# Ray0089/geometric-aware-dense-matching

Measured on AMD Instinct MI355X. Metric: rgbd_crops_per_sec_geomatch_fwd, higher is better.
Workload: dtype bf16x3/f32acc

## Files before the change

### geometric_aware_dense_matching_amd/csrc/gdm_image.hip

```cpp
#include "gdm_common.h"
#include "gdm_packed_act.h"

namespace {

__global__ __launch_bounds__(256) void upsample_bilinear_kernel(const float* __restrict__ in, int H, int W, int OH, int OW,
                                                                float rh, float rw, float* __restrict__ out)
{
    const long plane = blockIdx.y;
    const int qpr = (OW + 3) >> 2;
    const int q = blockIdx.x * 256 + threadIdx.x;
    if (q >= qpr * OH) return;
    const int oy = q / qpr;
    const int ox0 = (q - oy * qpr) * 4;
    const float sy = rh * (float)oy;
    const int y0 = (int)sy;
    const int y1 = y0 + (y0 < H - 1 ? 1 : 0);
    const float ly = sy - (float)y0, hy = 1.f - ly;
    const float* r0 = in + (plane * H + y0) * (long)W;
    const float* r1 = in + (plane * H + y1) * (long)W;
    float v[4];
#pragma unroll
    for (int j = 0; j < 4; ++j) {
        const int ox = min(ox0 + j, OW - 1);
        const float sx = rw * (float)ox;
        const int x0 = (int)sx;
        const int x1 = x0 + (x0 < W - 1 ? 1 : 0);
        const float lx = sx - (float)x0, hx = 1.f - lx;
        v[j] = hy * (hx * r0[x0] + lx * r0[x1]) + ly * (hx * r1[x0] + lx * r1[x1]);
    }
    float* o = out + (plane * OH + oy) * (long)OW + ox0;
    if (ox0 + 3 < OW && (((uintptr_t)o) & 15) == 0) {
        *reinterpret_cast<float4*>(o) = make_float4(v[0], v[1], v[2], v[3]);
    } else {
        for (int j = 0; j < 4 && ox0 + j < OW; ++j) o[j] = v[j];
    }
}

__device__ __forceinline__ void src_range(int i, int n_in, int n_out, float r, int& lo, int& hi)
{
    if (r <= 0.f) { lo = 0; hi = n_out - 1; return; }
    lo = max(0, (int)floorf((float)(i - 1) / r) - 1);
    hi = min(n_out - 1, (int)ceilf((float)(i + 1) / r) + 1);
}

__device__ __forceinline__ float tap_weight(int o, int i, int n_in, float r)
{
    const float sp = r * (float)o;
    const int i0 = min((int)sp, n_in - 1);
    const int i1 = i0 + (i0 < n_in - 1 ? 1 : 0);
    const float l = sp - (float)i0;
    return (i0 == i ? 1.f - l : 0.f) + (i1 == i ? l : 0.f);
}
// ... 528 lines not shown
            const int c = i - r * pw;
            const float* src = zb + (long)min(ys0 + r, H - 1) * W + min(xs0 + c, W - 1);
#pragma unroll
            for (int ch = 0; ch < 4; ++ch)
#pragma unroll
                for (int tap = 0; tap < 9; ++tap) patch[ch][tap][r][c] = src[((long)tap * Cout + ch) * plane_sz];
        }
        __syncthreads();
        if (live) {
#pragma unroll
            for (int dy = -1; dy <= 1; ++dy) {
                const int yy = oy + dy;
                if (yy < 0 || yy >= OH) continue;
                const float sy = rh * (float)yy;
                const int y0 = min((int)sy, H - 1);
                const float ly = sy - (float)y0, hy = 1.f - ly;
#pragma unroll
                for (int dx = -1; dx <= 1; ++dx) {
                    const int xx = ox + dx;
                    if (xx < 0 || xx >= OW) continue;
                    const int tap = (dy + 1) * 3 + (dx + 1);
                    const float sx = rw * (float)xx;
                    const int x0 = min((int)sx, W - 1);
                    const float lx = sx - (float)x0, hx = 1.f - lx;
                    const int xo = x0 - xs0, yo = y0 - ys0;
#pragma unroll
                    for (int ch = 0; ch < 4; ++ch) {
                        const float* r0 = &patch[ch][tap][yo][0];
                        const float* r1 = r0 + (U8_PW + 2);
                        const float top = fmaf(lx, r0[xo + 1], hx * r0[xo]);
                        const float bot = fmaf(lx, r1[xo + 1], hx * r1[xo]);
                        acc[4 * pass + ch] = fmaf(ly, bot, fmaf(hy, top, acc[4 * pass + ch]));
                    }
                }
            }
        }
    }
    if (!live) return;
    float v[8];
#pragma unroll
    for (int ch = 0; ch < 8; ++ch) {
        float o = acc[ch] * scale[c0 + ch] + shift[c0 + ch];
        if (ACT == 1) o = fmaxf(o, 0.f);
        if (ACT == 2) o = o > 0.f ? o : o * slope;
        v[ch] = o;
        out[(((long)b * Cout + c0 + ch) * OH + oy) * OW + ox] = o;
    }
    if (ypk) {
        const gdm_packed_map pm{Cout, OH, OW};
        gdm_packed_store8(ypk + pm.granule(b, c0 / GDM_PK_CHUNK, (c0 % GDM_PK_CHUNK) / 8, oy, ox), 0, pm.lo(), v);
    }
}

struct PspMaps {
    const float* y[4];
    int s[4];
    float sy[4], sx[4];
};

__global__ __launch_bounds__(256) void psp_combine_kernel(const float* __restrict__ g, PspMaps maps, const float* __restrict__ bias,
                                                          int C, int H, int W, float* __restrict__ out)
{
    const long plane = blockIdx.y;
    const int c = (int)(plane % C);
    const int hw = H * W;
    const float bc = bias ? bias[c] : 0.f;
    __shared__ float pm[4][64];
    {
        const int k = threadIdx.x >> 6, j = threadIdx.x & 63;
        if (j < maps.s[k] * maps.s[k]) pm[k][j] = maps.y[k][plane * maps.s[k] * maps.s[k] + j];
        __syncthreads();
    }
    for (int i0 = (blockIdx.x * 256 + threadIdx.x) * 4; i0 < hw; i0 += gridDim.x * 1024) {
        int oy = i0 / W, ox = i0 - oy * W;
        float v[4];
        const bool vec = i0 + 3 < hw;
        if (vec) {
            const float4 gv = *reinterpret_cast<const float4*>(g + plane * hw + i0);
            v[0] = gv.x; v[1] = gv.y; v[2] = gv.z; v[3] = gv.w;
        }
#pragma unroll
        for (int e = 0; e < 4; ++e) {
            if (i0 + e < hw) {
                float acc = (vec ? v[e] : g[plane * hw + i0 + e]) + bc;
#pragma unroll
                for (int k = 0; k < 4; ++k) {
                    const int S = maps.s[k];
                    const float* m = &pm[k][0];
                    const float fy = maps.sy[k] * (float)oy, fx = maps.sx[k] * (float)ox;
                    const int y0 = min((int)fy, S - 1), x0 = min((int)fx, S - 1);
                    const int y1 = y0 + (y0 < S - 1 ? 1 : 0), x1 = x0 + (x0 < S - 1 ? 1 : 0);
                    const float ly = fy - (float)y0, lx = fx - (float)x0;
                    acc += (1.f - ly) * ((1.f - lx) * m[y0 * S + x0] + lx * m[y0 * S + x1]) + ly * ((1.f - lx) * m[y1 * S + x0] + lx * m[y1 * S + x1]);
                }
                v[e] = fmaxf(acc, 0.f);
            }
            if (++ox == W) { ox = 0; ++oy; }
        }
        if (vec) *reinterpret_cast<float4*>(out + plane * hw + i0) = make_float4(v[0], v[1], v[2], v[3]);
        else
            for (int e = 0; e < 4 && i0 + e < hw; ++e) out[plane * hw + i0 + e] = v[e];
    }
}

__global__ __launch_bounds__(256) void psp_combine8_kernel(const float* __restrict__ g, PspMaps maps, const float* __restrict__ bias,
                                                           int C, int H, int W, float* __restrict__ out, unsigned char* __restrict__ ypk)
// ... 310 lines not shown
    GDM_CHECK_ARG(((uintptr_t)x & 15) == 0, "gdm_affine_act_maxk_hip: x must be 16-byte aligned");
    dim3 grid(gdm_cdiv(n, 256), (unsigned)planes);
    hipStream_t s = (hipStream_t)stream;
    gdm_dispatch_int<3>(act, [&](auto A) {
        hipLaunchKernelGGL(affine_act_maxk_kernel<decltype(A)::value>, grid, dim3(256), 0, s, x, scale, shift, C, n, K / 4, slope, out);
    });
    return gdm_launch_status("affine_act_maxk_kernel");
}

extern "C" int gdm_prelu1_hip(const float* x, const float* slope, long n, float* y, void* stream)
{
    GDM_CHECK_ARG(x && slope && y, "gdm_prelu1_hip: NULL pointer");
    GDM_CHECK_ARG(n >= 4 && n % 4 == 0 && (((uintptr_t)x | (uintptr_t)y) & 15) == 0, "gdm_prelu1_hip: n=%ld must be a multiple of 4 and the pointers 16-byte aligned", n);
    long blocks = gdm_cdiv(n / 4, 256);
    if (blocks > 8192) blocks = 8192;
    hipLaunchKernelGGL(prelu1_fwd_kernel, dim3((unsigned)blocks), dim3(256), 0, (hipStream_t)stream, (const float4*)x, slope, n / 4, (float4*)y);
    return gdm_launch_status("prelu1_fwd_kernel");
}

extern "C" int gdm_prelu1_bwd_hip(const float* x, const float* grad_out, const float* slope, long n, float* grad_x, float* grad_slope, void* stream)
{
    GDM_CHECK_ARG(x && grad_out && slope && grad_x && grad_slope, "gdm_prelu1_bwd_hip: NULL pointer");
    GDM_CHECK_ARG(n >= 4 && n % 4 == 0 && (((uintptr_t)x | (uintptr_t)grad_out | (uintptr_t)grad_x) & 15) == 0, "gdm_prelu1_bwd_hip: n=%ld must be a multiple of 4 and the pointers 16-byte aligned", n);
    long blocks = gdm_cdiv(n / 4, 256);
    if (blocks > 4096) blocks = 4096;
    hipLaunchKernelGGL(prelu1_bwd_kernel, dim3((unsigned)blocks), dim3(256), 0, (hipStream_t)stream, (const float4*)x, (const float4*)grad_out, slope,
                       n / 4, (float4*)grad_x, grad_slope);
    return gdm_launch_status("prelu1_bwd_kernel");
}

extern "C" int gdm_affine_act_hip(const float* x, const float* scale, const float* shift, const float* res, const float* res_scale,
                                  const float* res_shift, long planes, int C, long inner, int act, float slope, float* y, void* stream)
{
    GDM_CHECK_ARG(x && scale && shift && y, "gdm_affine_act_hip: NULL pointer");
    GDM_CHECK_ARG(planes >= 1 && planes <= 65535 && C >= 1 && inner >= 4 && inner % 4 == 0, "gdm_affine_act_hip: planes=%ld C=%d inner=%ld (inner %% 4 == 0, planes <= 65535)", planes, C, inner);
    GDM_CHECK_ARG(act >= 0 && act <= 2, "gdm_affine_act_hip: act=%d", act);
    GDM_CHECK_ARG((((uintptr_t)x | (uintptr_t)y | (uintptr_t)res) & 15) == 0, "gdm_affine_act_hip: pointers must be 16-byte aligned");
    const long inner4 = inner / 4;
    int gx = gdm_cdiv(inner4, 256);
    if (gx > 64) gx = 64;
    dim3 grid(gx, (unsigned)planes);
    hipStream_t s = (hipStream_t)stream;
    const bool has = res != nullptr, aff = res_scale != nullptr && res_shift != nullptr;
    gdm_dispatch_int<3>(act, [&](auto A) {
        gdm_dispatch_int<3>(!has ? 0 : aff ? 2 : 1, [&](auto R) {
            constexpr int RM = decltype(R)::value;
            hipLaunchKernelGGL((affine_act_kernel<decltype(A)::value, RM != 0, RM == 2>), grid, dim3(256), 0, s, x, scale, shift, res, res_scale,
                               res_shift, C, inner4, slope, y);
        });
    });
    return gdm_launch_status("affine_act_kernel");
}

extern "C" int gdm_upconv3x3_gather2_hip(const float* z, const float* scale, const float* shift, int B, int Cout, int H, int W,
                                         int OH, int OW, int act, float slope, float* out, void* outpk, void* stream)
{
    GDM_CHECK_ARG(z && scale && shift && out && outpk, "gdm_upconv3x3_gather2_hip: NULL pointer");
    GDM_CHECK_ARG(B >= 1 && Cout >= 8 && (long)B * (Cout / 8) <= 65535 && H >= 1 && W >= 1 && OH >= 1 && OW >= 1,
                  "gdm_upconv3x3_gather2_hip: bad shape B=%d Cout=%d %dx%d -> %dx%d", B, Cout, H, W, OH, OW);
    GDM_CHECK_ARG(act >= 0 && act <= 2 && gdm_packed_out_ok(Cout, outpk),
                  "gdm_upconv3x3_gather2_hip: act=%d / packed output needs Cout = 64 or a multiple of 128 and a 16-byte aligned buffer (Cout=%d)", act, Cout);
    const float rh = scale_ac(H, OH), rw = scale_ac(W, OW);
    GDM_CHECK_ARG((int)(rh * (U8_H + 1)) + 3 <= U8_PH && (int)(rw * (U8_W + 1)) + 3 <= U8_PW,
                  "gdm_upconv3x3_gather2_hip: scale factors %g x %g too large for the LDS tile (the x2 stages of PSPUpsample fit)", rh, rw);
    hipStream_t s = (hipStream_t)stream;
    dim3 grid(gdm_cdiv(OW, U8_W), gdm_cdiv(OH, U8_H), B * (Cout / 8));
    gdm_dispatch_int<3>(act, [&](auto A) {
        hipLaunchKernelGGL(upconv3x3_gather8_kernel<decltype(A)::value>, grid, dim3(256), 0, s, z, scale, shift, Cout, H, W, OH, OW, rh, rw, slope, out,
                           (unsigned char*)outpk);
    });
    return gdm_launch_status("upconv3x3_gather8_kernel");
}

extern "C" int gdm_upconv3x3_gather_hip(const float* z, const float* scale, const float* shift, int B, int Cout, int H, int W,
                                        int OH, int OW, int act, float slope, float* out, void* stream)
{
    GDM_CHECK_ARG(z && scale && shift && out, "gdm_upconv3x3_gather_hip: NULL pointer");
    GDM_CHECK_ARG(B >= 1 && Cout >= 1 && (long)B * Cout <= 65535 && H >= 1 && W >= 1 && OH >= 1 && OW >= 1,
                  "gdm_upconv3x3_gather_hip: bad shape B=%d Cout=%d %dx%d -> %dx%d", B, Cout, H, W, OH, OW);
    GDM_CHECK_ARG(act >= 0 && act <= 2, "gdm_upconv3x3_gather_hip: act=%d", act);
    hipStream_t s = (hipStream_t)stream;
    const float rh = scale_ac(H, OH), rw = scale_ac(W, OW);
    const bool lds_ok = (int)(rh * (UT_H + 1)) + 3 <= UP_PH && (int)(rw * (UT_W + 1)) + 3 <= UP_PW && (long)B * Cout <= 65535;
    if (lds_ok) {
        dim3 grid(gdm_cdiv(OW, UT_W), gdm_cdiv(OH, UT_H), B * Cout);
        gdm_dispatch_int<3>(act, [&](auto A) {
            hipLaunchKernelGGL(upconv3x3_gather_lds_kernel<decltype(A)::value>, grid, dim3(256), 0, s, z, scale, shift, Cout, H, W, OH, OW, rh, rw, slope, out);
        });
        return gdm_launch_status("upconv3x3_gather_lds_kernel");
    }
    const int quads = ((OW + 3) / 4) * OH;
    dim3 grid(gdm_cdiv(quads, 256), B * Cout);
    gdm_dispatch_int<3>(act, [&](auto A) {
        hipLaunchKernelGGL(upconv3x3_gather_kernel<decltype(A)::value>, grid, dim3(256), 0, s, z, scale, shift, Cout, H, W, OH, OW, rh, rw, slope, out);
    });
    return gdm_launch_status("upconv3x3_gather_kernel");
}

extern "C" int gdm_upconv3x3_gather_bwd_hip(const float* grad_out, int B, int Cout, int H, int W, int OH, int OW, float* grad_z, void* stream)
{
    GDM_CHECK_ARG(grad_out && grad_z, "gdm_upconv3x3_gather_bwd_hip: NULL pointer");
    GDM_CHECK_ARG(B >= 1 && Cout >= 1 && H >= 1 && W >= 1 && OH >= 1 && OW >= 1 && (long)B * 9 * Cout <= 65535,
                  "gdm_upconv3x3_gather_bwd_hip: bad shape B=%d Cout=%d (B*9*Cout <= 65535)", B, Cout);
    const float rh = scale_ac(H, OH), rw = scale_ac(W, OW);
    if (rh > 0.f && rw > 0.f && (int)ceilf((TL + 1) / rh) + 7 <= UB_P && (int)ceilf((TL + 1) / rw) + 7 <= UB_P) {
        dim3 grid3(gdm_cdiv(H, TL) * gdm_cdiv(W, TL), (unsigned)(B * Cout));
        hipLaunchKernelGGL(upconv3x3_gather_bwd_lds_kernel, grid3, dim3(256), 0, (hipStream_t)stream, grad_out, Cout, H, W, OH, OW, rh, rw, grad_z);
        return gdm_launch_status("upconv3x3_gather_bwd_lds_kernel");
    }
    dim3 grid(gdm_cdiv(H, TL) * gdm_cdiv(W, TL), (unsigned)(B * 9 * Cout));
    hipLaunchKernelGGL(upconv3x3_gather_bwd_kernel, grid, dim3(256), 0, (hipStream_t)stream, grad_out, Cout, H, W, OH, OW,
                       scale_ac(H, OH), scale_ac(W, OW), grad_z);
    return gdm_launch_status("upconv3x3_gather_bwd_kernel");
}

extern "C" int gdm_psp_combine2_hip(const float* g, const float* y1, int s1, const float* y2, int s2, const float* y3, int s3,
                                    const float* y4, int s4, const float* bias, int B, int C, int H, int W, float* out, void* outpk,
                                    void* stream)
{
    GDM_CHECK_ARG(g && y1 && y2 && y3 && y4 && out, "gdm_psp_combine2_hip: NULL pointer");
    GDM_CHECK_ARG(B >= 1 && C >= 1 && (long)B * C <= 65535 && H >= 1 && W >= 1 && s1 >= 1 && s2 >= 1 && s3 >= 1 && s4 >= 1,
                  "gdm_psp_combine2_hip: bad shape");
    GDM_CHECK_ARG(s1 <= 8 && s2 <= 8 && s3 <= 8 && s4 <= 8, "gdm_psp_combine2_hip: prior maps up to 8x8 (the reference uses 1, 2, 3, 6)");
    PspMaps maps;
    maps.y[0] = y1; maps.y[1] = y2; maps.y[2] = y3; maps.y[3] = y4;
    maps.s[0] = s1; maps.s[1] = s2; maps.s[2] = s3; maps.s[3] = s4;
    for (int k = 0; k < 4; ++k) {
        maps.sy[k] = H > 1 ? (float)(maps.s[k] - 1) / (float)(H - 1) : 0.f;
        maps.sx[k] = W > 1 ? (float)(maps.s[k] - 1) / (float)(W - 1) : 0.f;
    }
    GDM_CHECK_ARG(((long)H * W) % 4 == 0 && (((uintptr_t)g | (uintptr_t)out) & 15) == 0, "gdm_psp_combine2_hip: H*W must be a multiple of 4 and the maps 16-byte aligned");
    int gx = gdm_cdiv((long)H * W, 1024);
    if (gx > 16) gx = 16;
    if (outpk) {
        GDM_CHECK_ARG(W % 4 == 0 && gdm_packed_out_ok(C, outpk),
                      "gdm_psp_combine2_hip: packed output needs C = 64 or a multiple of 128, W %% 4 == 0 and a 16-byte aligned buffer (C=%d W=%d)", C, W);
        hipLaunchKernelGGL(psp_combine8_kernel, dim3(gx, B * C / 8), dim3(256), 0, (hipStream_t)stream, g, maps, bias, C, H, W, out,
// ... 116 lines not shown
```

### geometric_aware_dense_matching_amd/ops.py

```python
import collections
import ctypes
import functools
import os

import torch

from . import _lib, settings
from ._lib import KnnJob, call, check
from .derived import derived

MATCH_BF16X3 = _lib.GDM_MATCH_BF16X3
MATCH_F32 = _lib.GDM_MATCH_F32


def _stream():
    return torch.cuda.current_stream().cuda_stream


_side_streams = {}


def side_stream(device, which=0):
    key = (device.index if device.index is not None else torch.cuda.current_device(), which)
    st = _side_streams.get(key)
# ... 946 lines not shown
        return None
    group = bn.process_group if bn.process_group is not None else dist.group.WORLD
    return group if dist.get_world_size(group) >= settings.SYNCBN_MIN_WORLD else None


def bn_train_supported(x, bn):
    if not (settings.USE_FUSED_BN_TRAIN and bn.training and x.is_cuda and x.dtype == torch.float32 and x.dim() >= 3 and x.is_contiguous()):
        return False
    if type(bn) not in (torch.nn.BatchNorm1d, torch.nn.BatchNorm2d) and not (settings.USE_FUSED_SYNCBN and type(bn) is torch.nn.SyncBatchNorm):
        return False
    if not bn.affine or bn.momentum is None or not bn.track_running_stats:
        return False
    B, C = x.shape[0], x.shape[1]
    inner = x.numel() // max(B * C, 1)
    return B * C <= 65535 and inner >= 4 and inner % 4 == 0 and x.data_ptr() % 16 == 0 and B * inner > 1


def batch_norm_act_train(x, bn, act=ACT_NONE, slope=0.0):
    y = _BatchNormAct.apply(x, bn.weight, bn.bias, bn.running_mean, bn.running_var, bn.eps, bn.momentum, act, slope, _sync_group(bn))
    if bn.num_batches_tracked is not None:
        if _bn_counters is not None:
            _bn_counters.append(bn.num_batches_tracked)
        else:
            bn.num_batches_tracked.add_(1)
    return y


_bn_counters = None


class batched_bn_counters:

    def __enter__(self):
        global _bn_counters
        self.prev, _bn_counters = _bn_counters, []
        return self

    def __exit__(self, *exc):
        global _bn_counters
        pending, _bn_counters = _bn_counters, self.prev
        if pending:
            torch._foreach_add_(pending, 1)
        return False


def upconv3x3_gather(z, scale, shift, cout, out_size, act=ACT_NONE, slope=0.0, packed=False):
    z = _dev(z, torch.float32, "z")
    B, c9, H, W = z.shape
    assert c9 == 9 * cout
    OH, OW = int(out_size[0]), int(out_size[1])
    out = torch.empty((B, cout, OH, OW), dtype=torch.float32, device=z.device)
    if packed and packed_out_supported(B, cout, OH, OW, grid_groups=True) and (OH, OW) == (2 * H, 2 * W):
        opk = _packed_out(B, cout, OH, OW, z.device)
        call("gdm_upconv3x3_gather2_hip", z, scale, shift, B, cout, H, W, OH, OW, act, float(slope), out, opk.buf)
        return carry_packed(out, opk)
    call("gdm_upconv3x3_gather_hip", z, scale, shift, B, cout, H, W, OH, OW, act, float(slope), out)
    return out


def upconv_fused64_pack_weight(weight):
    w = _dev(weight.detach(), torch.float32, "weight")
    if tuple(w.shape) != (64, 64, 3, 3):
        raise ValueError("upconv_fused64_pack_weight: weight must be [64,64,3,3], got %s" % (tuple(w.shape),))
    L = _lib.lib()
    wpk = torch.empty(L.gdm_upconv_fused64_weight_bytes(), dtype=torch.uint8, device=w.device)
    call("gdm_upconv_fused64_pack_weight_hip", w, wpk)
    return wpk


def upconv_fused64(x, wpk, scale, shift, out_size, act=0, slope=0.0):
    x = _dev(x, torch.float32, "x")
    B, C, H, W = x.shape
    OH, OW = int(out_size[0]), int(out_size[1])
    out = torch.empty((B, C, OH, OW), dtype=torch.float32, device=x.device)
    call("gdm_upconv_fused64_hip", x, wpk, scale, shift, B, C, H, W, OH, OW, act, float(slope), out)
    return out


class _UpconvGather(torch.autograd.Function):

    @staticmethod
    def forward(ctx, z, bias, cout, OH, OW):
        z = z.contiguous()
        B, c9, H, W = z.shape
        ones = torch.ones(cout, dtype=torch.float32, device=z.device)
        shift = bias.detach().contiguous() if bias is not None else torch.zeros(cout, dtype=torch.float32, device=z.device)
        out = torch.empty((B, cout, OH, OW), dtype=torch.float32, device=z.device)
        call("gdm_upconv3x3_gather_hip", z, ones, shift, B, cout, H, W, OH, OW, ACT_NONE, 0.0, out)
        ctx.shape = (B, cout, H, W, OH, OW)
        ctx.has_bias = bias is not None
        return out

    @staticmethod
    def backward(ctx, go):
        B, cout, H, W, OH, OW = ctx.shape
        go = go.contiguous()
        gz = torch.empty((B, 9 * cout, H, W), dtype=torch.float32, device=go.device)
        call("gdm_upconv3x3_gather_bwd_hip", go, B, cout, H, W, OH, OW, gz)
        return gz, (channel_sum(go) if ctx.has_bias else None), None, None, None


def upconv3x3_gather_train(z, bias, cout, out_size):
    z = _dev(z, torch.float32, "z")
    assert z.shape[1] == 9 * cout
    return _UpconvGather.apply(z, bias, cout, int(out_size[0]), int(out_size[1]))


def wx(w2d, x3):
    if torch.is_grad_enabled() and (w2d.requires_grad or x3.requires_grad) and x3.is_cuda and x3.dtype == torch.float32:
        return _WxTrain.apply(x3.contiguous(), w2d.contiguous())
    return torch.bmm(w2d.unsqueeze(0).expand(x3.shape[0], -1, -1), x3)


OPERAND_LIMIT = 1 << 31


def operands_fit(*nbytes):
    return all(0 < n < OPERAND_LIMIT for n in nbytes)


def _require_fit(who, what, args, act_bytes, weight_bytes=None):
    if not operands_fit(act_bytes, *(() if weight_bytes is None else (weight_bytes,))):
        raise ValueError("%s: %s needs packed activations of %d bytes%s; a packed operand must be above 0 and below 2 GiB (%d bytes)"
                         % (who, what % args, act_bytes, "" if weight_bytes is None else " and packed weights of %d bytes" % weight_bytes,
                            OPERAND_LIMIT))


def _map_bytes(B, C, H, W):
    return _lib.lib().gdm_conv3x3_act_bytes(B, C, H, W)


def _wgrad_parts(nchunk, tiles):
    parts = 1
    for d in range(1, nchunk + 1):
        if nchunk % d == 0 and d * tiles <= 320 and nchunk // d >= 4:
            parts = d
    return parts


def _wgrad_packed(who, x, go, taps, parts=None):
    B, Cin, Cout = x.shape[0], x.shape[1], go.shape[1]
# ... 1260 lines not shown
```

### geometric_aware_dense_matching_amd/settings.py

```python
import os


def _flag(name, default="1"):
    return os.environ.get(name, default) != "0"


USE_MFMA_CONV = _flag("GDM_MFMA_CONV")
USE_MFMA_CONV_TRAIN = _flag("GDM_MFMA_CONV_TRAIN")
USE_MFMA_GEMM = _flag("GDM_MFMA_GEMM")
USE_FUSED_UPCONV = _flag("GDM_FUSED_UPCONV")
USE_LOWRES_UPCONV_TRAIN = _flag("GDM_LOWRES_UPCONV_TRAIN")
USE_SPLIT_PSP_TRAIN = _flag("GDM_SPLIT_PSP_TRAIN")
USE_FUSED_LFA = _flag("GDM_FUSED_LFA")
USE_GROUPED_SPLINE = _flag("GDM_GROUPED_SPLINE")
USE_FUSED_BN_TRAIN = _flag("GDM_FUSED_BN_TRAIN")
USE_FUSED_SYNCBN = _flag("GDM_FUSED_SYNCBN")
USE_FUSED_MATCH_LOSS = _flag("GDM_FUSED_MATCH_LOSS")
USE_SIDE_STREAMS = _flag("GDM_SIDE_STREAMS", "0")
USE_SPARSE_FINAL = _flag("GDM_SPARSE_FINAL")
USE_FUSED_HEADS = _flag("GDM_FUSED_HEADS")
USE_MFMA_STRIDED = _flag("GDM_MFMA_STRIDED")
USE_POINTWISE = _flag("GDM_POINTWISE")
USE_OWN_STEM = _flag("GDM_OWN_STEM")
USE_GEMM_CONV1X1_TRAIN = _flag("GDM_GEMM_CONV1X1_TRAIN")
USE_MFMA_WGRAD = _flag("GDM_MFMA_WGRAD")
USE_MFMA_GEMM_TRAIN = _flag("GDM_MFMA_GEMM_TRAIN")
USE_GATHERED_FINAL = _flag("GDM_GATHERED_FINAL")
USE_DIRECT_WGRAD = _flag("GDM_DIRECT_WGRAD")
USE_FUSED_ADAM = _flag("GDM_FUSED_ADAM")
USE_POINTWISE_TRAIN = _flag("GDM_POINTWISE_TRAIN")
USE_POINT_CHAIN = _flag("GDM_POINT_CHAIN")
USE_PSP_JOBS = _flag("GDM_PSP_JOBS")
USE_PACKED_PRODUCERS = _flag("GDM_PACKED_PRODUCERS")
MESH_FORK_LATE = os.environ.get("GDM_MESH_FORK_LATE", "1") != "0"
PACK_MESH_ROWS = os.environ.get("GDM_PACK_MESH_ROWS", "1") != "0"
SPLINE_LDS_WEIGHTS = os.environ.get("GDM_SPLINE_LDS_WEIGHTS", "1") != "0"
HEADS_MATCH_ROWS = os.environ.get("GDM_HEADS_MATCH_ROWS", "1") != "0"
SIDE_PARTS = os.environ.get("GDM_SIDE_PARTS", "mesh,point,pyr").split(",")
STATIC_MATCH_ROWS = _flag("GDM_STATIC_MATCH_ROWS", "0")
UPCONV_MIN_CIN = int(os.environ.get("GDM_UPCONV_MIN_CIN", "0"))
SYNCBN_MIN_WORLD = 2

ALL_SWITCHES = ("USE_MFMA_CONV", "USE_MFMA_CONV_TRAIN", "USE_MFMA_GEMM", "USE_FUSED_UPCONV", "USE_LOWRES_UPCONV_TRAIN",
                "USE_SPLIT_PSP_TRAIN", "USE_FUSED_LFA", "USE_GROUPED_SPLINE", "USE_FUSED_BN_TRAIN", "USE_FUSED_SYNCBN",
                "USE_FUSED_MATCH_LOSS", "USE_SIDE_STREAMS", "USE_SPARSE_FINAL", "USE_FUSED_HEADS", "USE_MFMA_STRIDED", "USE_POINTWISE", "USE_OWN_STEM", "USE_GEMM_CONV1X1_TRAIN", "USE_MFMA_WGRAD", "USE_MFMA_GEMM_TRAIN", "USE_GATHERED_FINAL", "USE_DIRECT_WGRAD", "USE_PSP_JOBS", "USE_POINT_CHAIN", "USE_POINTWISE_TRAIN")
SPLIT_BF16_SWITCHES = ("USE_MFMA_CONV", "USE_MFMA_GEMM", "USE_FUSED_UPCONV", "USE_SPARSE_FINAL", "USE_FUSED_HEADS", "USE_MFMA_STRIDED",
                       "USE_OWN_STEM")
```

### include/gdm.h

```cpp
#ifndef GDM_H
#define GDM_H

#include <stddef.h>
#include <stdint.h>

#ifdef __cplusplus
extern "C" {
#endif

#define GDM_EINVAL (-1)
#define GDM_ENOMEM (-2)

const char* gdm_last_error(void);
int gdm_version(void);


void gdm_knn_batch(const float* batch_data, size_t batch_size, size_t npts, size_t dim,
                   const float* queries, size_t nqueries, size_t K, long* batch_indices);

int gdm_knn_batch_hip(const float* support, const float* query, int B, int S, int Q, int K,
                      int32_t* idx, float* d2, void* stream);

typedef struct gdm_knn_job {
    const float* support;
// ... 151 lines not shown
                         const int32_t* best_idx, const uint8_t* mask, int B, int N, int M, double* out, void* stream);

int gdm_kabsch_solve_hip(const double* stats, int B, int min_points, float* RT, uint8_t* valid, void* stream);

int gdm_kabsch_stats_w_hip(const float* scene_xyz, long scene_bstride, int pt_stride, int ch_stride, const float* model_xyz,
                           const int32_t* best_idx, const float* target, const float* weight, const uint8_t* mask, int B, int N,
                           int M, double* out, int32_t* count, void* stream);
int gdm_kabsch_solve_w_hip(const double* stats, const int32_t* count, int B, int min_points, float* RT, uint8_t* valid, void* stream);

#define GDM_RANSAC_MAX_H 4096
size_t gdm_ransac_workspace_bytes(int B, int N, int H);
int gdm_ransac_pose_hip(const float* scene_xyz, long scene_bstride, int pt_stride, int ch_stride, const float* model_xyz,
                        const int32_t* best_idx, const uint8_t* mask, const double* stats, int B, int N, int M, int H,
                        float match_err, double fix_percent, uint32_t seed, int min_points, void* workspace, size_t workspace_bytes,
                        float* RT, uint8_t* valid, int32_t* counts, int32_t* winner, void* stream);

size_t gdm_consensus_workspace_bytes(int B, int N, int seeds);
int gdm_consensus_pose_hip(const float* scene_xyz, long scene_bstride, int pt_stride, int ch_stride, const float* model_xyz,
                           const int32_t* best_idx, const uint8_t* mask, int B, int N, int M, int seeds, float tau, float inlier_dist,
                           int min_points, void* workspace, size_t workspace_bytes, float* RT, uint8_t* valid, int32_t* score,
                           int32_t* degree, int32_t* seed_idx, float* hyp_RT, int32_t* counts, int32_t* winner, void* stream);

int gdm_icp_transform_hip(const float* scene_xyz, long scene_bstride, int pt_stride, int ch_stride, const float* RT, int B, int N,
                          float* query, void* stream);
int gdm_icp_update_hip(const float* scene_xyz, long scene_bstride, int pt_stride, int ch_stride, const float* model_xyz,
                       const int32_t* nn, const float* d2, const uint8_t* mask, int B, int N, int M, float reject_dist,
                       double tolerance, int min_points, float* RT, uint8_t* active, int32_t* iters, double* err, void* stream);

int gdm_icp_plane_update_hip(const float* scene_nrm, long scene_bstride, int pt_stride, int ch_stride, const float* query,
                             const float* model_xyz, const float* model_nrm, const int32_t* nn, const float* d2, const uint8_t* mask,
                             int B, int N, int M, float reject_dist, double normal_gate, double huber_delta, double tolerance,
                             int min_points, double pivot_min, float* RT, uint8_t* active, int32_t* iters, double* err,
                             int32_t* status, int32_t* n_pairs, void* stream);

#define GDM_TARGETS_MIN_M 4
size_t gdm_targets_workspace_bytes(int B, int N, int M);
int gdm_hpr_visible_hip(const float* model_xyz, long model_bstride, const float* RT, const float* cam_center, int B, int M,
                        void* workspace, size_t workspace_bytes, double* flipped, uint8_t* visible, void* stream);
int gdm_pose_targets_hip(const float* cld, long cld_bstride, int pt_stride, int ch_stride, const uint8_t* labels, const float* RT,
                         const float* model_xyz, long model_bstride, const uint8_t* visible, int B, int N, int M, double dist_thresh,
                         void* workspace, size_t workspace_bytes, uint8_t* labels_out, int32_t* match_idx, uint8_t* visible_flag,
                         uint8_t* valid, void* stream);

int gdm_affine_act_maxk_hip(const float* x, const float* scale, const float* shift, long planes, int C, long n, int K, int act,
                            float slope, float* out, void* stream);

int gdm_prelu1_hip(const float* x, const float* slope, long n, float* y, void* stream);
int gdm_prelu1_bwd_hip(const float* x, const float* grad_out, const float* slope, long n, float* grad_x, float* grad_slope, void* stream);

int gdm_affine_act_hip(const float* x, const float* scale, const float* shift, const float* res, const float* res_scale,
                       const float* res_shift, long planes, int C, long inner, int act, float slope, float* y, void* stream);

int gdm_upconv3x3_gather_hip(const float* z, const float* scale, const float* shift, int B, int Cout, int H, int W,
                             int OH, int OW, int act, float slope, float* out, void* stream);
int gdm_upconv3x3_gather2_hip(const float* z, const float* scale, const float* shift, int B, int Cout, int H, int W,
                              int OH, int OW, int act, float slope, float* out, void* outpk, void* stream);
int gdm_upconv3x3_gather_bwd_hip(const float* grad_out, int B, int Cout, int H, int W, int OH, int OW, float* grad_z, void* stream);
size_t gdm_upconv_fused64_weight_bytes(void);
int gdm_upconv_fused64_pack_weight_hip(const float* w, void* wpk, void* stream);
int gdm_upconv_fused64_hip(const float* x, const void* wpk, const float* scale, const float* shift, int B, int C, int H, int W,
                           int OH, int OW, int act, float slope, float* out, void* stream);

int gdm_psp_combine2_hip(const float* g, const float* y1, int s1, const float* y2, int s2, const float* y3, int s3,
                         const float* y4, int s4, const float* bias, int B, int C, int H, int W, float* out, void* outpk, void* stream);
int gdm_gather_add_affine_act2_hip(const float* x, const float* t, const int32_t* idx, const float* scale, const float* shift,
                                   int B, int C, int n, int m, int act, float slope, float* y, void* y_packed, int W, void* stream);
int gdm_conv1x1_gather_add_act2_hip(const float* x, const float* wt, const float* t, const int32_t* idx, const float* scale,
                                    const float* shift, int B, int C, int n, long m, int act, float slope, int pixel_major,
                                    float* y, void* stream);
int gdm_conv64_gather_add_act_mfma2_hip(const float* x, const void* wpk, const float* t, const int32_t* idx, const float* scale,
                                        const float* shift, int B, int n, long m, int act, float slope, int pixel_major,
                                        int t_point_major, float* y, void* ypk, int W, void* stream);
int gdm_conv64_gather_add_final_hip(const float* x, const void* wpk, const float* t, const int32_t* idx, const float* scale,
                                    const float* shift, int B, int n, long m, int act, float slope, const float* wft,
                                    const float* fbias, float* out, void* stream);

size_t gdm_conv3x3_act_bytes(int B, int Cin, int H, int W);
size_t gdm_conv3x3_weight_bytes(int Cout, int Cin);
int gdm_conv3x3_pack_weight_hip(const float* w, int Cout, int Cin, void* wpk, void* stream);
int gdm_conv3x3_pack_act_hip(const float* x, int B, int Cin, int H, int W, void* xpk, void* stream);
int gdm_conv3x3_packed_hip(const void* xpk, const void* wpk, const float* scale, const float* shift, const float* res,
                           int B, int Cin, int Cout, int H, int W, int act, float* out, void* stream);
int gdm_conv3x3_strided_hip(const void* xpk, const void* wpk, const float* scale, const float* shift, const float* res,
                            int B, int Cin, int Cout, int H, int W, int stride, int act, float* out, void* outpk, void* stream);
int gdm_conv1x1_strided_hip(const void* xpk, const void* wpk, const float* scale, const float* shift,
                            int B, int Cin, int Cout, int H, int W, int stride, int act, float* out, void* stream);
int gdm_conv1x1_gather_add_hip(const void* xpk, const void* wpk, const int32_t* gidx, const float* gt, int gn, const float* scale,
                               const float* shift, int B, int Cin, int Cout, int H, int W, int act, float* out, void* outpk, void* stream);

int gdm_affine_relu_maxpool_hip(const float* x, const float* scale, const float* shift, int B, int C, int H, int W, float* y, void* stream);
int gdm_conv1x1_logsoftmax_hip(const float* x, const float* w, const float* bias, int B, int C, long hw, float* out, void* stream);
int gdm_pack_rows64_hip(const float* w, int R, void* out, void* stream);
int gdm_upconv_final_points_hip(const float* xpm, const int32_t* choose, const void* wpk, const float* scale, const float* shift,
                                int act, float slope, const void* wfpk, const float* fbias, int B, int H, int W, int OH, int OW,
                                int N, float* out, void* stream);
int gdm_psp_pools_hip(const float* x, long planes, int H, int W, float* o1, float* o2, float* o3, float* o6, void* stream);
int gdm_psp_pools_bwd_hip(const float* g1, const float* g2, const float* g3, const float* g6, long planes, int H, int W,
                          float* grad_x, void* stream);

size_t gdm_conv1x1_weight_bytes(int Cout, int Cin);
int gdm_conv1x1_pack_weight_hip(const float* w, int Cout, int Cin, void* wpk, void* stream);
int gdm_conv_pack_weight_dgrad_hip(const float* w, int Cout, int Cin, int taps, void* wpk, void* stream);
int gdm_conv1x1_packed_hip(const void* xpk, const void* wpk, const float* scale, const float* shift,
                           int B, int Cin, int Cout, int H, int W, int act, int pixel_major, float* out, void* stream);

int gdm_depth_to_xyz_hip(const float* depth, const float* K, const int32_t* origin, int B, int H, int W, int S,
                         float* out, void* stream);

#define GDM_NORMALS_MAX_K 64
// ... 155 lines not shown
```

Baseline: 5407.

## Add full-row LDS tiled upconv3x3 gather kernels for exact x2 upsampling

Adds two new upconv3x3 gather kernels that stage whole input row windows for all nine taps into LDS using vectorized 16-byte loads. The next channel group's loads are software-pipelined behind the current compute, and a dispatcher picks these kernels for exact 2x upsampling with small widths. The packed eight-channel path is enabled by a default-on setting. The non-packed path always passes 0, so the four-channel rows kernel never runs from Python. This aims to cut redundant global gathers and per-tile halo overhead, at the cost of large LDS use per block, which may limit occupancy.

```diff
diff --git a/geometric_aware_dense_matching_amd/csrc/gdm_image.hip b/geometric_aware_dense_matching_amd/csrc/gdm_image.hip
--- a/geometric_aware_dense_matching_amd/csrc/gdm_image.hip
+++ b/geometric_aware_dense_matching_amd/csrc/gdm_image.hip
@@ -1,3 +1,4 @@
+#include <climits>
 #include "gdm_common.h"
 #include "gdm_packed_act.h"
 
@@ -632,6 +633,237 @@
     }
 }
 
+#ifdef __HIP_DEVICE_COMPILE__
+#define UR_NO_PACKED_F32 __attribute__((target("no-packed-fp32-ops")))
+#else
+#define UR_NO_PACKED_F32
+#endif
+__device__ __forceinline__ UR_NO_PACKED_F32 void ur_barrier()
+{
+    __builtin_amdgcn_fence(__ATOMIC_RELEASE, "workgroup");
+    __builtin_amdgcn_s_barrier();
+    __builtin_amdgcn_fence(__ATOMIC_ACQUIRE, "workgroup");
+}
+constexpr int UR_LAST = 1 << 30;
+
+template <int NLD, int NT, int NCH>
+__device__ __forceinline__ UR_NO_PACKED_F32 void rowfill_plan(int ph, int H, int W, int ys0, int Cout, unsigned plane_sz, int stride, unsigned (&g)[NLD], int (&l)[NLD])
+{
+    const int W4 = W >> 2, n = 9 * NCH * ph * W4;
+    const unsigned inv_w4 = ((1u << 20) + W4 - 1) / W4, inv_ph = ((1u << 20) + ph - 1) / ph;
+#pragma unroll
+    for (int k = 0; k < NLD; ++k) {
+        const int i = threadIdx.x + k * NT;
+        const int row = (int)(((unsigned)i * inv_w4) >> 20), c4 = i - row * W4;
+        const int p = (int)(((unsigned)row * inv_ph) >> 20), r = row - p * ph;
+        const int tap = p / NCH, ch = p - tap * NCH;
+        const bool is = i < n;
+        g[k] = is ? (unsigned)(tap * Cout + ch) * plane_sz + (unsigned)(min(ys0 + r, H - 1) * W + 4 * c4) : 0u;
+        l[k] = is ? (row * stride + 4 * c4) | (c4 == W4 - 1 ? UR_LAST : 0) : -1;
+    }
+}
+template <int NLD>
+__device__ __forceinline__ UR_NO_PACKED_F32 void rowfill_load(const float* __restrict__ zq, const unsigned (&g)[NLD], gdm_f32x4 (&v)[NLD])
+{
+#pragma unroll
+    for (int k = 0; k < NLD; ++k) v[k] = *reinterpret_cast<const gdm_f32x4*>(zq + g[k]);
+}
+template <int NLD>
+__device__ __forceinline__ UR_NO_PACKED_F32 void rowfill_store(float* patch, const int (&l)[NLD], const gdm_f32x4 (&v)[NLD])
+{
+#pragma unroll
+    for (int k = 0; k < NLD; ++k) {
+        if (l[k] >= 0) {
+            const int o = l[k] & (UR_LAST - 1);
+            *reinterpret_cast<gdm_f32x4*>(patch + o) = v[k];
+            if (l[k] & UR_LAST) patch[o + 4] = v[k][3];
+        }
+    }
+}
+__device__ __forceinline__ UR_NO_PACKED_F32 void rowfill_window(int oy_t, int TH, int H, int OH, float rh, int& ys0, int& ph)
+{
+    ys0 = min((int)(rh * (float)max(oy_t - 1, 0)), H - 1);
+    ph = min((int)(rh * (float)min(oy_t + TH, OH - 1)), H - 1) - ys0 + 2;
+}
+
+constexpr int R8_TH = 8, R8_PH = 7, R8_NLD = 8, R8_MAXW = 32, R8_LDS = 36 * R8_PH * (R8_MAXW + 4);
+
+template <int ACT>
+__global__ __launch_bounds__(256) UR_NO_PACKED_F32 void upconv3x3_rows8_kernel(const float* __restrict__ z, const float* __restrict__ scale,
+                                                                                const float* __restrict__ shift, int Cout, int H, int W, int OH, int OW,
+                                                                                float rh, float rw, float slope, float* __restrict__ out,
+                                                                                unsigned char* __restrict__ ypk)
+{
+    __shared__ __attribute__((aligned(16))) float patch[R8_LDS];
+    const int groups = Cout / 8;
+    const int b = blockIdx.y / groups, c0 = (blockIdx.y - b * groups) * 8;
+    const int oy_t = blockIdx.x * R8_TH;
+    int ys0, ph;
+    rowfill_window(oy_t, R8_TH, H, OH, rh, ys0, ph);
+    const int stride = W + 4;
+    const unsigned plane_sz = (unsigned)(H * W);
+    unsigned g[R8_NLD];
+    int l[R8_NLD];
+    rowfill_plan<R8_NLD, 256, 4>(ph, H, W, ys0, Cout, plane_sz, stride, g, l);
+    const float* zq = z + ((long)b * 9 * Cout + c0) * plane_sz;
+    gdm_f32x4 v[R8_NLD];
+    rowfill_load(zq, g, v);
+    int oy[2], ox[2];
+    bool live[2];
+#pragma unroll
+    for (int k = 0; k < 2; ++k) {
+        const int p = threadIdx.x + 256 * k;
+        const int row = p / OW;
+        oy[k] = oy_t + row, ox[k] = p - row * OW;
+        live[k] = row < R8_TH && oy[k] < OH;
+    }
+    float acc[2][8];
+#pragma unroll
+    for (int k = 0; k < 2; ++k)
+#pragma unroll
+        for (int ch = 0; ch < 8; ++ch) acc[k][ch] = 0.f;
+#pragma unroll
+    for (int pass = 0; pass < 2; ++pass) {
+        if (pass) ur_barrier();
+        rowfill_store(patch, l, v);
+        ur_barrier();
+        if (pass == 0) rowfill_load(zq + 4 * (long)plane_sz, g, v);
+#pragma unroll
+        for (int k = 0; k < 2; ++k) {
+            if (!live[k]) continue;
+#pragma unroll
+            for (int dy = -1; dy <= 1; ++dy) {
+                const int yy = oy[k] + dy;
+                if (yy < 0 || yy >= OH) continue;
+                const float sy = rh * (float)yy;
+                const int y0 = min((int)sy, H - 1);
+                const float ly = sy - (float)y0, hy = 1.f - ly;
+#pragma unroll
+                for (int dx = -1; dx <= 1; ++dx) {
+                    const int xx = ox[k] + dx;
+                    if (xx < 0 || xx >= OW) continue;
+                    const int tap = (dy + 1) * 3 + (dx + 1);
+                    const float sx = rw * (float)xx;
+                    const int x0 = min((int)sx, W - 1);
+                    const float lx = sx - (float)x0, hx = 1.f - lx;
+                    const float* rt = patch + ((tap * 4) * ph + (y0 - ys0)) * stride + x0;
+#pragma unroll
+                    for (int ch = 0; ch < 4; ++ch) {
+                        const float* r0 = rt + ch * ph * stride;
+                        const float* r1 = r0 + stride;
+                        const float top = fmaf(lx, r0[1], hx * r0[0]);
+                        const float bot = fmaf(lx, r1[1], hx * r1[0]);
+                        acc[k][4 * pass + ch] = fmaf(ly, bot, fmaf(hy, top, acc[k][4 * pass + ch]));
+                    }
+                }
+            }
+        }
+    }
+    const gdm_packed_map pm{Cout, OH, OW};
+#pragma unroll
+    for (int k = 0; k < 2; ++k) {
+        if (!live[k]) continue;
+        float o8[8];
+#pragma unroll
+        for (int ch = 0; ch < 8; ++ch) {
+            float o = acc[k][ch] * scale[c0 + ch] + shift[c0 + ch];
+            if (ACT == 1) o = fmaxf(o, 0.f);
+            if (ACT == 2) o = o > 0.f ? o : o * slope;
+            o8[ch] = o;
+            out[(((long)b * Cout + c0 + ch) * OH + oy[k]) * OW + ox[k]] = o;
+        }
+        if (ypk) gdm_packed_store8(ypk + pm.granule(b, c0 / GDM_PK_CHUNK, (c0 % GDM_PK_CHUNK) / 8, oy[k], ox[k]), 0, pm.lo(), o8);
+    }
+}
+
+constexpr int RP_TH = 16, RP_PH = 11, RP_NLD = 7, RP_NC = 4, RP_MAXW = 72, RP_LDS = 9 * RP_PH * (RP_MAXW + 4);
+static_assert(RP_TH * 16 == 256, "a thread's tile row is threadIdx.x >> 4");
+
+template <int ACT>
+__global__ __launch_bounds__(256) UR_NO_PACKED_F32 void upconv3x3_rows_kernel(const float* __restrict__ z, const float* __restrict__ scale,
+                                                                               const float* __restrict__ shift, int Cout, int H, int W, int OH, int OW,
+                                                                               float rh, float rw, float slope, float* __restrict__ out)
+{
+    __shared__ __attribute__((aligned(16))) float patch[RP_LDS];
+    const int cgroups = (Cout + RP_NC - 1) / RP_NC;
+    const int b = blockIdx.y / cgroups, c0 = (blockIdx.y - b * cgroups) * RP_NC;
+    const int nc = min(RP_NC, Cout - c0);
+    const int oy_t = blockIdx.x * RP_TH;
+    int ys0, ph;
+    rowfill_window(oy_t, RP_TH, H, OH, rh, ys0, ph);
+    const int stride = W + 4;
+    const unsigned plane_sz = (unsigned)(H * W);
+    unsigned g[RP_NLD];
+    int l[RP_NLD];
+    rowfill_plan<RP_NLD, 256, 1>(ph, H, W, ys0, Cout, plane_sz, stride, g, l);
+    const float* zc = z + ((long)b * 9 * Cout + c0) * plane_sz;
+    gdm_f32x4 v[RP_NLD];
+    rowfill_load(zc, g, v);
+    const int Q = OW >> 2, nxb = (Q + 15) >> 4;
+    const int oy = oy_t + (threadIdx.x >> 4);
+    for (int ci = 0; ci < nc; ++ci) {
+        if (ci) ur_barrier();
+        rowfill_store(patch, l, v);
+        ur_barrier();
+        if (ci + 1 < nc) rowfill_load(zc + (long)(ci + 1) * plane_sz, g, v);
+        const int co = c0 + ci;
+        const float a = scale[co], sh = shift[co];
+        for (int xb = 0; xb < nxb; ++xb) {
+            const int ox0 = (xb * 16 + (threadIdx.x & 15)) * 4;
+            if (oy >= OH || ox0 >= OW) continue;
+            int cx0[6];
+            float clx[6], chx[6];
+            bool cok[6];
+#pragma unroll
+            for (int j = 0; j < 6; ++j) {
+                const int ox = ox0 - 1 + j;
+                cok[j] = ox >= 0 && ox < OW;
+                const float sx = rw * (float)min(max(ox, 0), OW - 1);
+                const int x0 = min((int)sx, W - 1);
+                cx0[j] = x0;
+                clx[j] = sx - (float)x0;
+                chx[j] = 1.f - clx[j];
+            }
+            float acc[4] = {0.f, 0.f, 0.f, 0.f};
+#pragma unroll
+            for (int dy = -1; dy <= 1; ++dy) {
+                const int yy = oy + dy;
+                if (yy < 0 || yy >= OH) continue;
+                const float sy = rh * (float)yy;
+                const int y0 = min((int)sy, H - 1);
+                const float ly = sy - (float)y0, hy = 1.f - ly;
+#pragma unroll
+                for (int dx = -1; dx <= 1; ++dx) {
+                    const int tap = (dy + 1) * 3 + (dx + 1);
+                    const float* r0 = patch + (tap * ph + (y0 - ys0)) * stride;
+                    const float* r1 = r0 + stride;
+#pragma unroll
+                    for (int j = 0; j < 4; ++j) {
+                        const int c = j + dx + 1;
+                        if (cok[c]) {
+                            const float lx = clx[c], hx = chx[c];
+                            const int xo = cx0[c];
+                            const float top = fmaf(lx, r0[xo + 1], hx * r0[xo]);
+                            const float bot = fmaf(lx, r1[xo + 1], hx * r1[xo]);
+                            acc[j] = fmaf(ly, bot, fmaf(hy, top, acc[j]));
+                        }
+                    }
+                }
+            }
+            float o4[4];
+#pragma unroll
+            for (int j = 0; j < 4; ++j) {
+                float o = acc[j] * a + sh;
+                if (ACT == 1) o = fmaxf(o, 0.f);
+                if (ACT == 2) o = o > 0.f ? o : o * slope;
+                o4[j] = o;
+            }
+            const gdm_f32x4 ov = {o4[0], o4[1], o4[2], o4[3]};
+            *reinterpret_cast<gdm_f32x4*>(out + (((long)b * Cout + co) * OH + oy) * OW + ox0) = ov;
+        }
+    }
+}
+
 struct PspMaps {
     const float* y[4];
     int s[4];
@@ -1048,8 +1280,24 @@
     return gdm_launch_status("affine_act_kernel");
 }
 
+enum { GDM_UPCONV_DIRECT = 0, GDM_UPCONV_LDS = 1, GDM_UPCONV_EIGHT = 2, GDM_UPCONV_ROWS = 3, GDM_UPCONV_ROWS8 = 4 };
+extern "C" int gdm_upconv3x3_gather_form(const void* z, const void* out, int B, int Cout, int H, int W, int OH, int OW, int eight,
+                                         int row_fills)
+{
+    if (B < 1 || Cout < 1 || H < 1 || W < 1 || OH < 1 || OW < 1) return -1;
+    const float rh = scale_ac(H, OH), rw = scale_ac(W, OW);
+    const bool rows = row_fills && OH == 2 * H && OW == 2 * W && W % 4 == 0 && ((uintptr_t)z & 15) == 0 && 9L * Cout * H * W <= INT_MAX;
+    if (eight) {
+        if (Cout % 8 || !((int)(rh * (U8_H + 1)) + 3 <= U8_PH && (int)(rw * (U8_W + 1)) + 3 <= U8_PW)) return -1;
+        return rows && W <= R8_MAXW ? GDM_UPCONV_ROWS8 : GDM_UPCONV_EIGHT;
+    }
+    if (rows && W <= RP_MAXW && ((uintptr_t)out & 15) == 0 && (long)B * gdm_cdiv(Cout, RP_NC) <= 65535) return GDM_UPCONV_ROWS;
+    const bool lds_ok = (int)(rh * (UT_H + 1)) + 3 <= UP_PH && (int)(rw * (UT_W + 1)) + 3 <= UP_PW && (long)B * Cout <= 65535;
+    return lds_ok ? GDM_UPCONV_LDS : GDM_UPCONV_DIRECT;
+}
+
 extern "C" int gdm_upconv3x3_gather2_hip(const float* z, const float* scale, const float* shift, int B, int Cout, int H, int W,
-                                         int OH, int OW, int act, float slope, float* out, void* outpk, void* stream)
+                                         int OH, int OW, int act, float slope, float* out, void* outpk, int row_fills, void* stream)
 {
     GDM_CHECK_ARG(z && scale && shift && out && outpk, "gdm_upconv3x3_gather2_hip: NULL pointer");
     GDM_CHECK_ARG(B >= 1 && Cout >= 8 && (long)B * (Cout / 8) <= 65535 && H >= 1 && W >= 1 && OH >= 1 && OW >= 1,
@@ -1057,9 +1305,18 @@
     GDM_CHECK_ARG(act >= 0 && act <= 2 && gdm_packed_out_ok(Cout, outpk),
                   "gdm_upconv3x3_gather2_hip: act=%d / packed output needs Cout = 64 or a multiple of 128 and a 16-byte aligned buffer (Cout=%d)", act, Cout);
     const float rh = scale_ac(H, OH), rw = scale_ac(W, OW);
-    GDM_CHECK_ARG((int)(rh * (U8_H + 1)) + 3 <= U8_PH && (int)(rw * (U8_W + 1)) + 3 <= U8_PW,
+    const int form = gdm_upconv3x3_gather_form(z, out, B, Cout, H, W, OH, OW, 1, row_fills);
+    GDM_CHECK_ARG(form >= 0,
                   "gdm_upconv3x3_gather2_hip: scale factors %g x %g too large for the LDS tile (the x2 stages of PSPUpsample fit)", rh, rw);
     hipStream_t s = (hipStream_t)stream;
+    if (form == GDM_UPCONV_ROWS8) {
+        dim3 grid(gdm_cdiv(OH, R8_TH), B * (Cout / 8));
+        gdm_dispatch_int<3>(act, [&](auto A) {
+            hipLaunchKernelGGL(upconv3x3_rows8_kernel<decltype(A)::value>, grid, dim3(256), 0, s, z, scale, shift, Cout, H, W, OH, OW, rh, rw, slope, out,
+                               (unsigned char*)outpk);
+        });
+        return gdm_launch_status("upconv3x3_rows8_kernel");
+    }
     dim3 grid(gdm_cdiv(OW, U8_W), gdm_cdiv(OH, U8_H), B * (Cout / 8));
     gdm_dispatch_int<3>(act, [&](auto A) {
         hipLaunchKernelGGL(upconv3x3_gather8_kernel<decltype(A)::value>, grid, dim3(256), 0, s, z, scale, shift, Cout, H, W, OH, OW, rh, rw, slope, out,
@@ -1069,7 +1326,7 @@
 }
 
 extern "C" int gdm_upconv3x3_gather_hip(const float* z, const float* scale, const float* shift, int B, int Cout, int H, int W,
-                                        int OH, int OW, int act, float slope, float* out, void* stream)
+                                        int OH, int OW, int act, float slope, float* out, int row_fills, void* stream)
 {
     GDM_CHECK_ARG(z && scale && shift && out, "gdm_upconv3x3_gather_hip: NULL pointer");
     GDM_CHECK_ARG(B >= 1 && Cout >= 1 && (long)B * Cout <= 65535 && H >= 1 && W >= 1 && OH >= 1 && OW >= 1,
@@ -1077,8 +1334,15 @@
     GDM_CHECK_ARG(act >= 0 && act <= 2, "gdm_upconv3x3_gather_hip: act=%d", act);
     hipStream_t s = (hipStream_t)stream;
     const float rh = scale_ac(H, OH), rw = scale_ac(W, OW);
-    const bool lds_ok = (int)(rh * (UT_H + 1)) + 3 <= UP_PH && (int)(rw * (UT_W + 1)) + 3 <= UP_PW && (long)B * Cout <= 65535;
-    if (lds_ok) {
+    const int form = gdm_upconv3x3_gather_form(z, out, B, Cout, H, W, OH, OW, 0, row_fills);
+    if (form == GDM_UPCONV_ROWS) {
+        dim3 grid(gdm_cdiv(OH, RP_TH), B * gdm_cdiv(Cout, RP_NC));
+        gdm_dispatch_int<3>(act, [&](auto A) {
+            hipLaunchKernelGGL(upconv3x3_rows_kernel<decltype(A)::value>, grid, dim3(256), 0, s, z, scale, shift, Cout, H, W, OH, OW, rh, rw, slope, out);
+        });
+        return gdm_launch_status("upconv3x3_rows_kernel");
+    }
+    if (form == GDM_UPCONV_LDS) {
         dim3 grid(gdm_cdiv(OW, UT_W), gdm_cdiv(OH, UT_H), B * Cout);
         gdm_dispatch_int<3>(act, [&](auto A) {
             hipLaunchKernelGGL(upconv3x3_gather_lds_kernel<decltype(A)::value>, grid, dim3(256), 0, s, z, scale, shift, Cout, H, W, OH, OW, rh, rw, slope, out);
diff --git a/geometric_aware_dense_matching_amd/ops.py b/geometric_aware_dense_matching_amd/ops.py
--- a/geometric_aware_dense_matching_amd/ops.py
+++ b/geometric_aware_dense_matching_amd/ops.py
@@ -1022,9 +1022,10 @@
     out = torch.empty((B, cout, OH, OW), dtype=torch.float32, device=z.device)
     if packed and packed_out_supported(B, cout, OH, OW, grid_groups=True) and (OH, OW) == (2 * H, 2 * W):
         opk = _packed_out(B, cout, OH, OW, z.device)
-        call("gdm_upconv3x3_gather2_hip", z, scale, shift, B, cout, H, W, OH, OW, act, float(slope), out, opk.buf)
+        call("gdm_upconv3x3_gather2_hip", z, scale, shift, B, cout, H, W, OH, OW, act, float(slope), out, opk.buf,
+             int(settings.UPCONV_ROW_FILLS))
         return carry_packed(out, opk)
-    call("gdm_upconv3x3_gather_hip", z, scale, shift, B, cout, H, W, OH, OW, act, float(slope), out)
+    call("gdm_upconv3x3_gather_hip", z, scale, shift, B, cout, H, W, OH, OW, act, float(slope), out, 0)
     return out
 
 
@@ -1056,7 +1057,7 @@
         ones = torch.ones(cout, dtype=torch.float32, device=z.device)
         shift = bias.detach().contiguous() if bias is not None else torch.zeros(cout, dtype=torch.float32, device=z.device)
         out = torch.empty((B, cout, OH, OW), dtype=torch.float32, device=z.device)
-        call("gdm_upconv3x3_gather_hip", z, ones, shift, B, cout, H, W, OH, OW, ACT_NONE, 0.0, out)
+        call("gdm_upconv3x3_gather_hip", z, ones, shift, B, cout, H, W, OH, OW, ACT_NONE, 0.0, out, 0)
         ctx.shape = (B, cout, H, W, OH, OW)
         ctx.has_bias = bias is not None
         return out
diff --git a/geometric_aware_dense_matching_amd/settings.py b/geometric_aware_dense_matching_amd/settings.py
--- a/geometric_aware_dense_matching_amd/settings.py
+++ b/geometric_aware_dense_matching_amd/settings.py
@@ -36,6 +36,7 @@
 PACK_MESH_ROWS = os.environ.get("GDM_PACK_MESH_ROWS", "1") != "0"
 SPLINE_LDS_WEIGHTS = os.environ.get("GDM_SPLINE_LDS_WEIGHTS", "1") != "0"
 HEADS_MATCH_ROWS = os.environ.get("GDM_HEADS_MATCH_ROWS", "1") != "0"
+UPCONV_ROW_FILLS = os.environ.get("GDM_UPCONV_ROW_FILLS", "1") != "0"
 SIDE_PARTS = os.environ.get("GDM_SIDE_PARTS", "mesh,point,pyr").split(",")
 STATIC_MATCH_ROWS = _flag("GDM_STATIC_MATCH_ROWS", "0")
 UPCONV_MIN_CIN = int(os.environ.get("GDM_UPCONV_MIN_CIN", "0"))
diff --git a/include/gdm.h b/include/gdm.h
--- a/include/gdm.h
+++ b/include/gdm.h
@@ -227,9 +227,10 @@
                        const float* res_shift, long planes, int C, long inner, int act, float slope, float* y, void* stream);
 
 int gdm_upconv3x3_gather_hip(const float* z, const float* scale, const float* shift, int B, int Cout, int H, int W,
-                             int OH, int OW, int act, float slope, float* out, void* stream);
+                             int OH, int OW, int act, float slope, float* out, int row_fills, void* stream);
 int gdm_upconv3x3_gather2_hip(const float* z, const float* scale, const float* shift, int B, int Cout, int H, int W,
-                              int OH, int OW, int act, float slope, float* out, void* outpk, void* stream);
+                              int OH, int OW, int act, float slope, float* out, void* outpk, int row_fills, void* stream);
+int gdm_upconv3x3_gather_form(const void* z, const void* out, int B, int Cout, int H, int W, int OH, int OW, int eight, int row_fills);
 int gdm_upconv3x3_gather_bwd_hip(const float* grad_out, int B, int Cout, int H, int W, int OH, int OW, float* grad_z, void* stream);
 size_t gdm_upconv_fused64_weight_bytes(void);
 int gdm_upconv_fused64_pack_weight_hip(const float* w, void* wpk, void* stream);
```

Result: no change. 5455, median of 6 (+0.9%).
